# wavelab/libwave

Measured on AMD Instinct MI355X. Metric: point-cloud registrations/sec (1M<->1M pts, ICP), higher is better.
Workload: dtype f32

## Files before the change

### libwave_amd/csrc/wm_bins.hpp

```cpp
#ifndef WM_BINS_HPP
#define WM_BINS_HPP

#include "wm_internal.hpp"

namespace wm {

constexpr int kBinCount = 64;
constexpr int kBinLimbs = 3;
constexpr int kBinComps = kAcc + 1;
constexpr int kBinStride = 32;
constexpr size_t kBinWords = (size_t) kBinCount * kBinLimbs * kBinStride;

__device__ __host__ inline long long bins_to_i64(double v) {
    const double d = v + 6755399441055744.0;
    long long bits;
    __builtin_memcpy(&bits, &d, sizeof(bits));
    return (bits & 0x000FFFFFFFFFFFFFll) - 0x0008000000000000ll;
}

__device__ __host__ inline void bins_split(double x, long long (&l)[kBinLimbs]) {
    const double t2 = trunc(x * 5.9604644775390625e-08);
    const double r1 = fma(-t2, 16777216.0, x);
    const double t1 = trunc(r1 * 65536.0);
    const double r0 = fma(-t1, 1.52587890625e-05, r1);
    const double t0 = trunc(r0 * 72057594037927936.0);
    l[2] = bins_to_i64(t2);
    l[1] = bins_to_i64(t1);
    l[0] = bins_to_i64(t0);
}

constexpr unsigned kBinPoison = kBinStride - 1;
__device__ __forceinline__ void bins_add(long long *bins, unsigned bin, unsigned comp, double x) {
    long long l[kBinLimbs];
    long long *p = bins + (size_t) bin * (kBinLimbs * kBinStride) + comp;
    if (!(fabs(x) < 4611686018427387904.0)) {
        (void) __hip_atomic_fetch_add(bins + (size_t) bin * (kBinLimbs * kBinStride) + kBinPoison, 1ll, __ATOMIC_RELAXED,
                                      __HIP_MEMORY_SCOPE_AGENT);
        return;
    }
    bins_split(x, l);
#pragma unroll
    for (int k = 0; k < kBinLimbs; ++k)
        (void) __hip_atomic_fetch_add(p + k * kBinStride, l[k], __ATOMIC_RELAXED, __HIP_MEMORY_SCOPE_AGENT);
}
__device__ __forceinline__ void bins_add_count(long long *bins, unsigned bin, unsigned comp, long long n) {
    (void) __hip_atomic_fetch_add(bins + (size_t) bin * (kBinLimbs * kBinStride) + comp, n, __ATOMIC_RELAXED, __HIP_MEMORY_SCOPE_AGENT);
}

__device__ __host__ inline double bins_value(long long L0, long long L1, long long L2);

template <int COMPS>
struct BinsLdsT {
    long long part[4][kBinLimbs * COMPS];
    double tot[COMPS];
    unsigned poison;
};
using BinsLds = BinsLdsT<kBinComps>;
template <int THREADS, int COMPS = kBinComps, int VALUES = kAcc>
__device__ __forceinline__ void bins_collect(long long *__restrict__ bins, BinsLdsT<COMPS> &B) {
    static_assert(COMPS < (int) kBinPoison && VALUES <= COMPS, "components below the poison word");
    constexpr int kBinComps = COMPS, kAcc = VALUES;
    constexpr int kWordsPerBin = kBinLimbs * kBinComps;
    constexpr int kGroups = THREADS >= 4 * kWordsPerBin ? 4 : 2;
    static_assert(THREADS >= kGroups * kWordsPerBin && kBinCount % kGroups == 0, "bins per thread group");
    constexpr int kPer = kBinCount / kGroups;
    const unsigned g = threadIdx.x / (unsigned) kWordsPerBin, j = threadIdx.x % (unsigned) kWordsPerBin;
    const unsigned limb = j / (unsigned) kBinComps, comp = j % (unsigned) kBinComps;
    if (threadIdx.x == 0) B.poison = 0u;
    if (g < (unsigned) kGroups) {
        long long v[kPer];
#pragma unroll
        for (int b = 0; b < kPer; ++b)
            v[b] = bins[((size_t) (g * kPer + b) * kBinLimbs + limb) * kBinStride + comp];
        long long t = 0;
#pragma unroll
        for (int b = 0; b < kPer; ++b) t += v[b];
        B.part[g][j] = t;
#pragma unroll
        for (int b = 0; b < kPer; ++b)
            bins[((size_t) (g * kPer + b) * kBinLimbs + limb) * kBinStride + comp] = 0ll;
    }
    __syncthreads();
    if (threadIdx.x < (unsigned) kBinCount) {
        long long *pw = bins + (size_t) threadIdx.x * (kBinLimbs * kBinStride) + kBinPoison;
        if (*pw != 0ll) {
            atomicOr(&B.poison, 1u);
            *pw = 0ll;
        }
    }
    if (threadIdx.x < (unsigned) kBinComps) {
        long long L[kBinLimbs];
#pragma unroll
        for (int l = 0; l < kBinLimbs; ++l) {
            long long t = 0;
#pragma unroll
            for (int gg = 0; gg < kGroups; ++gg) t += B.part[gg][l * kBinComps + threadIdx.x];
            L[l] = t;
        }
        B.tot[threadIdx.x] = threadIdx.x < (unsigned) kAcc ? bins_value(L[0], L[1], L[2]) : (double) L[0];
    }
    __syncthreads();
}

__device__ __host__ inline double bins_value(long long L0, long long L1, long long L2) {
    double term[6];
    const long long L[3] = {L2, L1, L0};
    const double scale[3] = {16777216.0, 1.52587890625e-05, 1.3877787807814457e-17};
    for (int k = 0; k < 3; ++k) {
        const long long hi = L[k] >> 32;
        const long long lo = L[k] - hi * 4294967296ll;
        term[2 * k] = (double) hi * 4294967296.0 * scale[k];
        term[2 * k + 1] = (double) lo * scale[k];
    }
    double s = 0.0, c = 0.0;
    for (int k = 0; k < 6; ++k) {
        const double t = s + term[k];
        const double bb = t - s;
        const double err = (s - (t - bb)) + (term[k] - bb);
        s = t;
        c += err;
    }
    return s + c;
}

}

#endif
```

### libwave_amd/csrc/wm_icp.hip

```cpp
#include "wm_internal.hpp"
#include "wm_icp_step.hpp"
#include "wm_pair_terms.hpp"
#include "wm_bins.hpp"
#include "wm_xchg.hpp"

#include <chrono>
#include <utility>
#include <vector>

#include <float.h>
#include <math.h>
#include <string.h>

#include <new>

namespace wm {

constexpr int kMaxStatBlocks = 256;
constexpr int kStatUnroll = 4;

template <int MODE>
__global__ void __launch_bounds__(kBlock)
    k_icp_stats(const float4 *__restrict__ src, unsigned n,
                const unsigned long long *__restrict__ keys, const float4 *__restrict__ tgt,
                const IcpDevState *__restrict__ st, double *__restrict__ partials, const int *__restrict__ rej) {
    if (st->done) return;
    const int rej_thr = rej ? *rej : 0x7FFFFFFF;
    double a[kAcc];
#pragma unroll
    for (int k = 0; k < kAcc; ++k) a[k] = 0.0;
    const bool slab_on = st->slab_on != 0;
    const float slab_lo = st->slab_lo, slab_hi = st->slab_hi;
    const unsigned stride = gridDim.x * kBlock;
    for (unsigned i0 = blockIdx.x * kBlock + threadIdx.x; i0 < n; i0 += kStatUnroll * stride) {
        float4 p4v[kStatUnroll], q4v[kStatUnroll];
        unsigned long long keyv[kStatUnroll];
#pragma unroll
        for (int u = 0; u < kStatUnroll; ++u) {
            const unsigned i = i0 + u * stride;
            const unsigned ic = i < n ? i : i0;
            p4v[u] = src[ic];
            keyv[u] = keys[ic];
            q4v[u] = tgt[ic];
        }
#pragma unroll
        for (int u = 0; u < kStatUnroll; ++u) {
            if (i0 + u * stride >= n) break;
            float fx, fy, fz;
            xform_pcl(st->Tf, p4v[u].x, p4v[u].y, p4v[u].z, fx, fy, fz);
            if (slab_on && !(fx >= slab_lo && fx < slab_hi)) continue;
            a[17] += 1.0;
            const unsigned long long key = keyv[u];
            if ((unsigned) key == kNoIdx) continue;
            if ((int) (unsigned) (key >> 32) > rej_thr) continue;
            icp_pair_terms<MODE>(fx, fy, fz, q4v[u].x, q4v[u].y, q4v[u].z, __uint_as_float((unsigned) (key >> 32)),
                                 [&](int k, double term) { a[k] += term; });
        }
    }
#pragma unroll
    for (int k = 0; k < kAcc; ++k)
#pragma unroll
        for (int off = 32; off > 0; off >>= 1) a[k] += __shfl_down(a[k], off);
    __shared__ double lds[kBlock / 64][kAcc];
    const int lane = threadIdx.x & 63, wave = threadIdx.x >> 6;
    if (lane == 0)
#pragma unroll
        for (int k = 0; k < kAcc; ++k) lds[wave][k] = a[k];
    __syncthreads();
    if (threadIdx.x < kAcc) {
        double s = 0;
        for (int w = 0; w < kBlock / 64; ++w) s += lds[w][threadIdx.x];
        partials[(size_t) blockIdx.x * kAcc + threadIdx.x] = s;
    }
}

constexpr int kPreRows = 128;
__global__ void __launch_bounds__(kBlock)
    k_reduce_rows(const double *__restrict__ partials, int rows, const IcpDevState *__restrict__ st,
                  double *__restrict__ out) {
    if (st->done) return;
    constexpr int kLanes = kBlock / kAcc;
    __shared__ double lds[kLanes][kAcc];
    const int c = threadIdx.x % kAcc, r = threadIdx.x / kAcc;
    const int r0 = blockIdx.x * kPreRows, r1 = min(r0 + kPreRows, rows);
    if (r < kLanes) {
        double v[(kPreRows + kLanes - 1) / kLanes];
        int k = 0;
#pragma unroll
        for (int b = r0 + r, u = 0; u < (kPreRows + kLanes - 1) / kLanes; b += kLanes, ++u, ++k)
            v[u] = b < r1 ? partials[(size_t) b * kAcc + c] : 0.0;
        double s = 0.0;
#pragma unroll
        for (int u = 0; u < (kPreRows + kLanes - 1) / kLanes; ++u) s += v[u];
        lds[r][c] = s;
    }
    __syncthreads();
    if (threadIdx.x < kAcc) {
        double t = 0.0;
#pragma unroll
        for (int l = 0; l < kLanes; ++l) t += lds[l][threadIdx.x];
        out[(size_t) blockIdx.x * kAcc + threadIdx.x] = t;
    }
}

__global__ void __launch_bounds__(kBlock)
    k_bins_solve(long long *__restrict__ bins, IcpDevState *st, unsigned long long *pub, int pub_slots) {
    __shared__ IcpDevState s_st;
    __shared__ BinsLds s_b;
    const unsigned long long t_start = clock64();
    static_assert(sizeof(IcpDevState) % 4 == 0, "word-wise staging");
    constexpr unsigned kWords = sizeof(IcpDevState) / 4;
    constexpr unsigned kStage = (kWords + kBlock - 1) / kBlock;
    unsigned stage[kStage];
#pragma unroll
    for (unsigned k = 0; k < kStage; ++k) {
        const unsigned w = threadIdx.x + k * kBlock;
        stage[k] = w < kWords ? reinterpret_cast<const unsigned *>(st)[w] : 0u;
    }
    bins_collect<kBlock>(bins, s_b);
#pragma unroll
    for (unsigned k = 0; k < kStage; ++k) {
        const unsigned w = threadIdx.x + k * kBlock;
        if (w < kWords) reinterpret_cast<unsigned *>(&s_st)[w] = stage[k];
    }
    __syncthreads();
    if (s_st.done) return;
    if (threadIdx.x == 0) {
        s_st.dbg[0] = t_start;
        s_st.dbg[1] = clock64();
        double a[kAcc], ex[kStatsLen];
#pragma unroll
        for (int k = 0; k < kAcc; ++k) a[k] = s_b.poison ? 0.0 : s_b.tot[k];
        expand_stats(s_st.mode, a, ex, s_st.changed_mask);
        s_st.local_handled = ex[kStatsLen - 1];
#pragma unroll
        for (int k = 0; k < kStatsLen; ++k) s_st.stats[k] = ex[k];
        s_st.dbg[2] = clock64();
        icp_apply_stats(&s_st, ex, (long long) s_b.tot[kAcc]);
        publish_step(&s_st, pub, pub_slots);
        s_st.dbg[3] = clock64();
    }
    __syncthreads();
    for (unsigned w = threadIdx.x; w < kWords; w += kBlock)
        reinterpret_cast<unsigned *>(st)[w] = reinterpret_cast<const unsigned *>(&s_st)[w];
}

template <int PHASES, int THREADS>
__global__ void __launch_bounds__(THREADS)
    k_reduce_solve(const double *__restrict__ partials, int nblocks, IcpDevState *st,
                   double *stats_io, unsigned long long *pub, int pub_slots, int blk_ext, XchgDev xd, long long *bins) {
    __shared__ IcpDevState s_st;
    const unsigned long long t_start = clock64();
    static_assert(sizeof(IcpDevState) % 4 == 0, "word-wise staging");
    constexpr unsigned kWords = sizeof(IcpDevState) / 4;
    constexpr unsigned kStage = (kWords + THREADS - 1) / THREADS;
    unsigned stage[kStage];
#pragma unroll
    for (unsigned k = 0; k < kStage; ++k) {
        const unsigned w = threadIdx.x + k * THREADS;
        stage[k] = w < kWords ? reinterpret_cast<const unsigned *>(st)[w] : 0u;
    }
    constexpr int kRows = THREADS / kAcc;
    constexpr int kGroups = 8;
    __shared__ double lds[kRows][kAcc];
    __shared__ double lds2[kGroups][kAcc];
    __shared__ double tot[kAcc];
    __shared__ BinsLds s_b;
    const bool from_bins = (PHASES & 1) && bins != nullptr;
    if (from_bins) {
        bins_collect<THREADS>(bins, s_b);
    } else if (PHASES & 1) {
        const int c = threadIdx.x % kAcc, r = threadIdx.x / kAcc;
        if (r < kRows) {
            constexpr int U = 16;
            double s[U];
#pragma unroll
            for (int u = 0; u < U; ++u) s[u] = 0.0;
            for (int b = r; b < nblocks; b += U * kRows) {
                double v[U];
#pragma unroll
                for (int u = 0; u < U; ++u) {
                    const int bb = b + u * kRows;
                    v[u] = bb < nblocks ? partials[(size_t) bb * kAcc + c] : 0.0;
                }
#pragma unroll
                for (int u = 0; u < U; ++u) s[u] += v[u];
            }
#pragma unroll
            for (int w = U / 2; w > 0; w >>= 1)
#pragma unroll
                for (int u = 0; u < w; ++u) s[u] += s[u + w];
            lds[r][c] = s[0];
        }
    }
#pragma unroll
    for (unsigned k = 0; k < kStage; ++k) {
        const unsigned w = threadIdx.x + k * THREADS;
        if (w < kWords) reinterpret_cast<unsigned *>(&s_st)[w] = stage[k];
    }
    if (from_bins) {
        if (threadIdx.x < (unsigned) kAcc) tot[threadIdx.x] = s_b.poison ? 0.0 : s_b.tot[threadIdx.x];
    } else if (PHASES & 1) {
        const int c = threadIdx.x % kAcc;
        __syncthreads();
        if (threadIdx.x < kGroups * kAcc) {
            const int g = threadIdx.x / kAcc;
            double t = 0.0;
            for (int sl = g; sl < kRows; sl += kGroups) t += lds[sl][c];
            lds2[g][c] = t;
        }
        __syncthreads();
        if (threadIdx.x < kAcc) {
            double t = 0.0;
#pragma unroll
            for (int g = 0; g < kGroups; ++g) t += lds2[g][threadIdx.x];
            tot[threadIdx.x] = t;
        }
    }
    __syncthreads();
    if (s_st.done) return;
    __shared__ unsigned s_uns;
    if (threadIdx.x < 64) {
        unsigned v = s_st.cert_unsettled[threadIdx.x];
        s_st.cert_unsettled[threadIdx.x] = 0u;
#pragma unroll
        for (int off = 32; off > 0; off >>= 1) v += (unsigned) __shfl_xor((int) v, off);
        if (threadIdx.x == 0) s_uns = from_bins ? (unsigned) s_b.tot[kAcc] : v;
    }
    if constexpr (PHASES == 7) {
        __shared__ double s_blk[kBlkLen], s_sum[kBlkLen];
        __shared__ unsigned s_half[kXMaxWorld * kXWords], s_ctl[2];
        if (threadIdx.x == 0) {
            double a[kAcc];
#pragma unroll
            for (int k = 0; k < kAcc; ++k) a[k] = tot[k];
            double ex[kStatsLen];
            expand_stats(s_st.mode, a, ex, s_st.changed_mask);
            s_st.local_handled = ex[kStatsLen - 1];
            ex[kStatsLen - 2] = s_st.stripe_finite;
#pragma unroll
            for (int k = 0; k < kStatsLen; ++k) s_blk[k] = ex[k];
            s_blk[kStatsLen] = (double) s_uns;
            s_blk[kStatsLen + 1] = 0.0;
        }
        __syncthreads();
        const bool arrived = xchg_allreduce<THREADS>(xd, s_blk, s_sum, s_half, s_ctl) && s_sum[kStatsLen + 1] == 0.0;
        if (threadIdx.x == 0) {
            s_st.dbg[0] = t_start;
            s_st.dbg[1] = clock64();
            if (!arrived) {
                s_st.xchg_failed = 1;
                s_st.done = 1;
                s_st.converged = 0;
                if (pub) __hip_atomic_store(pub, pack_done_word(1, s_st.iter), __ATOMIC_RELAXED, __HIP_MEMORY_SCOPE_SYSTEM);
            } else {
                double stats[kStatsLen];
#pragma unroll
                for (int k = 0; k < kStatsLen; ++k) stats[k] = s_st.stats[k] = s_sum[k];
                s_st.uns_global = 1;
                s_st.dbg[2] = clock64();
                icp_apply_stats(&s_st, stats, (long long) s_sum[kStatsLen]);
                if (stats_io)
                    for (int k = 0; k < kBlkLen; ++k) stats_io[k] = s_sum[k];
                publish_step(&s_st, pub, pub_slots);
            }
            s_st.dbg[3] = clock64();
        }
    } else if (threadIdx.x == 0) {
        s_st.dbg[0] = t_start;
        s_st.dbg[1] = clock64();
        if (PHASES & 1) {
            double a[kAcc];
#pragma unroll
            for (int k = 0; k < kAcc; ++k) a[k] = tot[k];
            double ex[kStatsLen];
            expand_stats(s_st.mode, a, ex, s_st.changed_mask);
            s_st.local_handled = ex[kStatsLen - 1];
#pragma unroll
            for (int k = 0; k < kStatsLen; ++k) s_st.stats[k] = ex[k];
            if (PHASES == 1 && stats_io) {
                ex[kStatsLen - 2] = s_st.stripe_finite;
#pragma unroll
                for (int k = 0; k < kStatsLen; ++k) stats_io[k] = ex[k];
                if (blk_ext) {
                    stats_io[kStatsLen] = (double) s_uns;
                    stats_io[kStatsLen + 1] = 0.0;
                }
            }
        } else if (stats_io) {
#pragma unroll
            for (int k = 0; k < kStatsLen; ++k) s_st.stats[k] = stats_io[k];
            s_st.uns_global = blk_ext ? 1 : 0;
        }
        if (PHASES & 2) {
            double stats[kStatsLen];
#pragma unroll
            for (int k = 0; k < kStatsLen; ++k) stats[k] = s_st.stats[k];
            s_st.dbg[2] = clock64();
            const long long uns_total = (PHASES == 2 && stats_io && blk_ext) ? (long long) stats_io[kStatsLen] : (long long) s_uns;
            icp_apply_stats(&s_st, stats, uns_total);
            publish_step(&s_st, pub, pub_slots);
        }
        s_st.dbg[3] = clock64();
    }
    __syncthreads();
    for (unsigned w = threadIdx.x; w < kWords; w += THREADS)
        reinterpret_cast<unsigned *>(st)[w] = reinterpret_cast<const unsigned *>(&s_st)[w];
}

__global__ void __launch_bounds__(kBlock) k_xchg_commit(IcpDevState *st, XchgDev xd) {
    __shared__ double s_blk[kBlkLen], s_sum[kBlkLen];
    __shared__ unsigned s_half[kXMaxWorld * kXWords], s_ctl[2];
    if (threadIdx.x < (unsigned) kBlkLen) s_blk[threadIdx.x] = 0.0;
    __syncthreads();
    if (threadIdx.x == 0) {
        s_blk[0] = st->xchg_failed ? 0.0 : 1.0;
        s_blk[kStatsLen + 1] = 1.0;
    }
    __syncthreads();
    const bool arrived = xchg_allreduce<kBlock>(xd, s_blk, s_sum, s_half, s_ctl);
    if (threadIdx.x == 0 && (!arrived || s_sum[0] != (double) xd.world || s_sum[kStatsLen + 1] != (double) xd.world)) {
        st->xchg_failed = 1;
        st->converged = 0;
    }
}

__global__ void __launch_bounds__(kBlock)
    k_unpack_corr(const float4 *__restrict__ src, unsigned n,
                  const unsigned long long *__restrict__ keys, int *__restrict__ match,
                  float *__restrict__ d2) {
    const unsigned i = blockIdx.x * kBlock + threadIdx.x;
    if (i >= n) return;
    const unsigned orig = __float_as_uint(src[i].w);
    const unsigned long long key = keys[i];
    const unsigned idx = (unsigned) key;
    match[orig] = idx == kNoIdx ? -1 : (int) idx;
    d2[orig] = __uint_as_float((unsigned) (key >> 32));
}

static int stat_blocks(size_t n) {
    size_t b = (n + kBlock - 1) / kBlock;
    if (b > kMaxStatBlocks) b = kMaxStatBlocks;
    if (b < 1) b = 1;
    return (int) b;
}

unsigned stat_rows(const wm_ctx *ctx) { return (unsigned) stat_blocks(ctx->n_src); }

int launch_stats(wm_ctx *ctx, int mode, const int *rej) {
    const unsigned n = (unsigned) ctx->n_src;
    const int nb = stat_blocks(n);
    const IcpDevState *st = ctx->d_state.as<IcpDevState>();
    if (mode == WM_ICP_SVD)
        hipLaunchKernelGGL(HIP_KERNEL_NAME(k_icp_stats<WM_ICP_SVD>), dim3(nb), dim3(kBlock), 0,
                           ctx->stream, ctx->src_sorted.as<float4>(), n,
                           ctx->keys.as<unsigned long long>(), ctx->match_pt.as<float4>(), st,
                           ctx->partials.as<double>(), rej);
    else
        hipLaunchKernelGGL(HIP_KERNEL_NAME(k_icp_stats<WM_ICP_GN6>), dim3(nb), dim3(kBlock), 0,
                           ctx->stream, ctx->src_sorted.as<float4>(), n,
                           ctx->keys.as<unsigned long long>(), ctx->match_pt.as<float4>(), st,
                           ctx->partials.as<double>(), rej);
    WM_HIP(ctx, hipGetLastError());
    return WM_OK;
}

int bins_ready(wm_ctx *ctx) {
    if (!ctx->bins.p || ctx->bins_dirty) {
        WM_HIP(ctx, ctx->bins.reserve(kBinWords * sizeof(long long)));
        WM_HIP(ctx, hipMemsetAsync(ctx->bins.p, 0, kBinWords * sizeof(long long), ctx->stream));
        ctx->bins_dirty = false;
    }
    return WM_OK;
// ... 816 lines not shown
```

### libwave_amd/csrc/wm_nn.hip

```cpp
#include "wm_nn_scan.hpp"

namespace wm {

template <int STATS, bool BAL, bool COST = false>
__global__ void __launch_bounds__(64) __attribute__((amdgpu_waves_per_eu(5, 5)))
    k_nn_grid(const LevelsDev lv, const float4 *__restrict__ src, unsigned n,
              IcpDevState *__restrict__ st, float thr_d2, unsigned long long *__restrict__ keys,
              float4 *__restrict__ match_pt, const float4 *__restrict__ tgt_orig,
              float r_light_cells, float lane_lf, float coop_lf, float r0_cells, unsigned chunk_sz,
              double *__restrict__ partials, unsigned *__restrict__ cost_out,
              unsigned long long *__restrict__ phase_out, long long *__restrict__ bins, float rmax) {
    const unsigned lane = threadIdx.x & 63u;
    const unsigned row_c = xcd_remap_chunked(blockIdx.x, max(chunk_sz, 1u)), row_e = xcd_remap(blockIdx.x, gridDim.x);
    const unsigned row = chunk_sz ? row_c : row_e;
    const unsigned i = row * 64u + lane;
    const bool active = i < n;
    const unsigned ic = min(i, n - 1u);
    const float4 p_e = src[ic];
    const unsigned long long prev_e = keys[ic];
    const float4 tp_e = match_pt[ic];
    const NnState S = nn_state(st);
    const int L = lv.n;
    float hl[kMaxLevels];
#pragma unroll
// ... 37 lines not shown
        if (prev != ~0ull) {
            const unsigned pidx = (unsigned) prev;
            r = rmax;
            if (pidx != kNoIdx) {
                const float d2b = canon_d2(qx, qy, qz, tp);
                if (d2b <= thr_d2) {
                    best = seeded = make_key(d2b, pidx);
                    bqx = tp.x;
                    bqy = tp.y;
                    bqz = tp.z;
                    r = fmaxf(__builtin_amdgcn_sqrtf(d2b) * 1.0001f + 1e-6f, 0.05f * h0);
                }
            }
        }
        r = fminf(r, rmax);
        heavy = r > r_light();
    }
    const unsigned long long prof_pro = COST ? clock64() : 0ull;
    if constexpr (BAL) {
        BalLds &L = s_hold.v;
        L.q[lane] = make_float4(qx, qy, qz, 0.f);
        L.seeded[lane] = seeded;
        L.bq[0][lane] = bqx;
        L.bq[1][lane] = bqy;
        L.bq[2][lane] = bqz;
        asm volatile("" ::: "memory");
        bool live = mine && !heavy;
        const bool allow_layered = true;
        bool probing = live && (unsigned) best == kNoIdx && r < rmax;
        if (__ballot(probing) != 0ull) {
            float rp = r0_cells * h0;
            for (int rung = 0; rung < 16 && __ballot(probing) != 0ull; ++rung) {
                int lp = 0;
#pragma unroll
                for (int k = 1; k < kMaxLevels; ++k) lp += (k < L_levels && hl[k] <= rp) ? 1 : 0;
                const GridDev g = lv.g[lp];
                unsigned cand;
                const bool empty = probe_box_empty(g, probing, qx, qy, qz, rp, cand);
                const bool hit = probing && !empty;
                const f4v ct = ((gp_f4) g.pts)[hit ? cand : 0u];
                if (hit) {
                    const float d2c = canon_d2v(qx, qy, qz, ct);
                    const float rc = fmaxf(__builtin_amdgcn_sqrtf(d2c) * 1.0001f + 1e-6f, 0.05f * h0);
                    if (d2c <= thr_d2 && rc <= r_light()) {
                        best = make_key(d2c, __float_as_uint(ct.w));
                        r = fminf(rc, rmax);
                    }
                }
                if (probing) {
                    if constexpr (COST) cost += ((cost >> 28) & 7u) < 7u ? 1u << 28 : 0u;
                    if (empty) {
                        r = nn_grow_radius(best, 0.f, r, rmax);
                        heavy = r > r_light();
                        live = !heavy;
                    }
                    probing = empty && live && r < rmax;
                }
                rp = fminf(2.0f * rp, rmax);
            }
        }
        for (int pass = 0; pass < 32 && __ballot(live) != 0ull; ++pass) {
            const int l = nn_level_for(hl, L_levels, lane_lf, r);
            const unsigned long long lv_mask = __ballot(live);
            const int l0 = __builtin_amdgcn_readlane(l, __ffsll((long long) lv_mask) - 1);
            float margin;
            if (__ballot(live && l != l0) == 0ull) {
                const GridDev g = lv.g[l0];
                best = scan_box_bal<COST, kBalRowChunk>(g, live, qx, qy, qz, r, best, &margin, L, lane, allow_layered, g.pts, cost, prof);
            } else {
                const GridDev g = lv.g[l];
                L.base[lane] = (unsigned long long) g.pts;
                best = scan_box_bal<COST, kBalRowChunk>(g, live, qx, qy, qz, r, best, &margin, L, lane, allow_layered, nullptr, cost, prof);
            }
            if (live) {
                if constexpr (COST) cost += ((cost >> 24) & 15u) < 15u ? 1u << 24 : 0u;
                const float bd2 = __uint_as_float((unsigned) (best >> 32));
                if (nn_certified(margin, bd2, thr_d2)) {
                    live = false;
                } else {
                    r = nn_grow_radius(best, bd2, r, rmax);
                    heavy = r > r_light();
                    live = !heavy;
                }
            }
        }
    } else if (mine) {
        for (int pass = 0; !heavy && pass < 32; ++pass) {
            const int l = nn_level_for(hl, L_levels, lane_lf, r);
            const GridDev g = lv.g[l];
            float margin;
            best = scan_box<COST>(g, qx, qy, qz, r, best, &margin, s_runs, lane, have_prev, cost);
            if constexpr (COST) cost += ((cost >> 24) & 15u) < 15u ? 1u << 24 : 0u;
            const float bd2 = __uint_as_float((unsigned) (best >> 32));
            if (nn_certified(margin, bd2, thr_d2)) break;
            r = nn_grow_radius(best, bd2, r, rmax);
            heavy = r > r_light();
        }
    }
    const unsigned long long prof_pass = COST ? clock64() : 0ull;
    unsigned long long todo = __ballot(heavy);
    const unsigned n_heavy = __popcll(todo);
    float seed = 0.f;
    while (todo) {
        const int sl = __ffsll((long long) todo) - 1;
        todo &= todo - 1;
        const float ux = rl_f(qx, sl), uy = rl_f(qy, sl), uz = rl_f(qz, sl);
        float ur = rl_f(r, sl);
        unsigned long long ub = ((unsigned long long) rl_u((unsigned) (best >> 32), sl) << 32) |
                                rl_u((unsigned) best, sl);
        if ((unsigned) ub == kNoIdx && seed > ur) ur = fminf(seed, rmax);
        for (int pass = 0; pass < 64; ++pass) {
            const int l = nn_level_for(hl, L_levels, coop_lf, ur);
            const GridDev g = lv.g[l];
            float margin;
            ub = coop_scan_box(g, ux, uy, uz, ur, ub, lane, &margin);
            const float bd2 = __uint_as_float((unsigned) (ub >> 32));
            if (nn_certified(margin, bd2, thr_d2)) break;
            if (ur >= rmax) break;
            ur = nn_grow_radius(ub, bd2, ur, rmax);
        }
        seed = ((unsigned) ub != kNoIdx) ? 1.25f * sqrtf(__uint_as_float((unsigned) (ub >> 32))) : ur;
        if ((int) lane == sl) best = ub;
    }
    const unsigned lane_e = __builtin_amdgcn_mbcnt_hi(~0u, __builtin_amdgcn_mbcnt_lo(~0u, 0u));
    const unsigned i_e = BAL ? row * 64u + lane_e : i;
    if constexpr (BAL) {
        asm volatile("" ::: "memory");
        BalLds &L = s_hold.v;
        seeded = L.seeded[lane_e];
        bqx = L.bq[0][lane_e];
        bqy = L.bq[1][lane_e];
        bqz = L.bq[2][lane_e];
    }
    if (mine) {
        st_u64(&keys[i_e], best);
        if (best != seeded && (unsigned) best != kNoIdx) {
            const f4v c = ((gp_f4) tgt_orig)[(unsigned) best];
            bqx = c.x;
            bqy = c.y;
            bqz = c.z;
        }
        if (!(best == seeded && (unsigned) best != kNoIdx))
            st_f4(&match_pt[i_e], bqx, bqy, bqz, __uint_as_float((unsigned) best));
    }
    if (lane == 0 && n_heavy) atomicAdd(&st->queue_count[1], n_heavy);
    const unsigned long long prof_store = COST ? clock64() : 0ull;
    if constexpr (COST) {
        if (active) cost_out[i_e] = mine ? (cost | (heavy ? 0x80000000u : 0u)) : 0u;
    }
    if constexpr (STATS >= 0) {
        double a[kAcc];
        icp_terms<STATS>(a, mine, (unsigned) best != kNoIdx, qx, qy, qz, bqx, bqy, bqz,
                         __uint_as_float((unsigned) (best >> 32)),
                         (unsigned) best != (unsigned) seeded && (i_e & st->changed_mask) == 0u);
        acc_halve<kAcc, 32>(a, lane);
        const int comp = acc_comp_of_lane(lane);
        if (comp >= 0) {
            if (bins) bins_add(bins, row % (unsigned) kBinCount, (unsigned) comp, a[0]);
            else st_f64(&partials[(size_t) row * kAcc + comp], a[0]);
        }
    }
    if constexpr (COST) {
        if (lane_e == 0 && phase_out) {
            const unsigned long long t_end = clock64();
            atomicAdd(&phase_out[0], prof[0]);
            atomicAdd(&phase_out[1], prof[1]);
            atomicAdd(&phase_out[2], prof[2]);
            atomicAdd(&phase_out[3], prof_pro - prof_start);
            atomicAdd(&phase_out[4], prof_pass - prof_pro);
            atomicAdd(&phase_out[5], prof_store - prof_pass);
            atomicAdd(&phase_out[6], t_end - prof_store);
            atomicAdd(&phase_out[7], 1ull);
        }
    }
}

constexpr int kBruteTile = 1024;

__global__ void __launch_bounds__(kBlock) k_init_keys(unsigned long long *keys, unsigned n,
                                                       const IcpDevState *st, float thr_d2) {
    if (st->done) return;
    const unsigned i = blockIdx.x * kBlock + threadIdx.x;
    if (i < n) keys[i] = make_key(thr_d2, kNoIdx);
}

__global__ void __launch_bounds__(kBlock)
    k_nn_brute(const float4 *__restrict__ tgt, unsigned m, const float4 *__restrict__ src,
               unsigned n, const IcpDevState *__restrict__ st, float thr_d2,
               unsigned long long *__restrict__ keys) {
    if (st->done) return;
    __shared__ float4 tile[kBruteTile];
    const unsigned i = blockIdx.x * kBlock + threadIdx.x;
    const unsigned per = (m + gridDim.y - 1) / gridDim.y;
    const unsigned m0 = blockIdx.y * per, m1 = min(m0 + per, m);
    float qx = 0, qy = 0, qz = 0;
    if (i < n) xform_pcl(st->Tf, src[i].x, src[i].y, src[i].z, qx, qy, qz);
    const bool mine = !(st->slab_on && !(qx >= st->slab_lo && qx < st->slab_hi));
    unsigned long long best = make_key(thr_d2, kNoIdx);
    for (unsigned t0 = m0; t0 < m1; t0 += kBruteTile) {
        const unsigned cnt = min((unsigned) kBruteTile, m1 - t0);
        __syncthreads();
        for (unsigned k = threadIdx.x; k < cnt; k += kBlock) tile[k] = tgt[t0 + k];
        __syncthreads();
        for (unsigned k = 0; k < cnt; ++k) {
            const float4 t = tile[k];
            const unsigned long long key = make_key(canon_d2(qx, qy, qz, t), __float_as_uint(t.w));
            best = key < best ? key : best;
        }
    }
    if (i < n && mine && best < make_key(thr_d2, kNoIdx)) atomicMin(&keys[i], best);
}

__global__ void __launch_bounds__(kBlock)
    k_fill_match(const unsigned long long *__restrict__ keys, unsigned n,
                 const float4 *__restrict__ tgt, const IcpDevState *__restrict__ st,
                 float4 *__restrict__ match_pt) {
    if (st->done) return;
    const unsigned i = blockIdx.x * kBlock + threadIdx.x;
    if (i >= n) return;
    const unsigned idx = (unsigned) keys[i];
    match_pt[i] = idx == kNoIdx ? make_float4(0.f, 0.f, 0.f, __uint_as_float(kNoIdx)) : tgt[idx];
}

static float threshold_below(double max_corr, bool strict) {
    const double m2 = max_corr * max_corr;
    if (!(m2 < 3.0e38)) return 3.0e38f;
    float f = (float) m2;
    if (strict ? (double) f >= m2 : (double) f > m2) f = nextafterf(f, 0.0f);
    return f;
}
float threshold_d2(double max_corr) { return threshold_below(max_corr, false); }
float threshold_d2_strict(double max_corr) { return threshold_below(max_corr, true); }

int nn_sums_target(wm_ctx *ctx, int stats_mode, bool use_bins, unsigned blocks, long long **bins, unsigned *rows_out) {
    *bins = nullptr;
    if (stats_mode >= 0 && use_bins) {
        if (!ctx->bins.p) return WM_ERR_STATE;
        *bins = ctx->bins.as<long long>();
    } else if (stats_mode >= 0) {
        WM_HIP(ctx, ctx->partials.reserve((size_t) blocks * kAcc * sizeof(double)));
        if (rows_out) *rows_out = blocks;
    }
    return WM_OK;
}

template <int STATS, bool BAL, bool COST = false>
static void launch_nn_grid_t(wm_ctx *ctx, unsigned blocks, float thr_d2, unsigned xcd_chunk, long long *bins = nullptr) {
    hipLaunchKernelGGL(HIP_KERNEL_NAME(k_nn_grid<STATS, BAL, COST>), dim3(blocks), dim3(64), 0, ctx->stream,
                       ctx->levels_dev, ctx->src_sorted.as<float4>(), (unsigned) ctx->n_src,
                       ctx->d_state.as<IcpDevState>(), thr_d2, ctx->keys.as<unsigned long long>(),
                       ctx->match_pt.as<float4>(), ctx->tgt_orig.as<float4>(), ctx->tune_r_light,
                       ctx->tune_lane_lf, ctx->tune_coop_lf, ctx->tune_r0, xcd_chunk, ctx->partials.as<double>(),
                       ctx->cost_log.p ? ctx->cost_log.as<unsigned>() + (size_t) ctx->cost_log_iter * ctx->n_src : nullptr,
                       ctx->phase_log.p ? ctx->phase_log.as<unsigned long long>() + 8 * (size_t) ctx->cost_log_iter : nullptr, bins,
                       sqrtf(thr_d2) * 1.0001f + 1e-6f);
}

int launch_nn_grid(wm_ctx *ctx, float thr_d2, hipEvent_t ev0, hipEvent_t ev1, hipEvent_t ev2,
                   int stats_mode, unsigned *rows_out, bool use_bins) {
    const unsigned n = (unsigned) ctx->n_src;
    if (rows_out) *rows_out = 0;
    if (n == 0) return WM_OK;
    unsigned blocks = (n + 63u) / 64u;
    blocks = (blocks + 7u) & ~7u;
    unsigned xcd_chunk = 0;
    if (ctx->tune_xcd_chunk > 0 && blocks >= 32u * (unsigned) ctx->tune_xcd_chunk) {
        xcd_chunk = (unsigned) ctx->tune_xcd_chunk;
        const unsigned m = 8u * xcd_chunk;
        blocks = (blocks + m - 1u) / m * m;
    }
    long long *bins = nullptr;
    const int rc = nn_sums_target(ctx, stats_mode, use_bins, blocks, &bins, rows_out);
    if (rc != WM_OK) return rc;
    const bool bal = ctx->tune_nn_balanced && ctx->n_tgt_input < (1u << 26) - 8u;
    if (ev0) WM_HIP(ctx, hipEventRecord(ev0, ctx->stream));
    if (stats_mode == WM_ICP_SVD && ctx->cost_log.p && ctx->cost_log_iter < ctx->cost_log_cap) {
        if (bal) launch_nn_grid_t<WM_ICP_SVD, true, true>(ctx, blocks, thr_d2, xcd_chunk, bins);
        else launch_nn_grid_t<WM_ICP_SVD, false, true>(ctx, blocks, thr_d2, xcd_chunk, bins);
        ctx->cost_log_iter++;
    } else if (stats_mode < 0) {
        if (bal) launch_nn_grid_t<-1, true>(ctx, blocks, thr_d2, xcd_chunk);
        else launch_nn_grid_t<-1, false>(ctx, blocks, thr_d2, xcd_chunk);
    } else if (stats_mode == WM_ICP_SVD) {
        if (bal) launch_nn_grid_t<WM_ICP_SVD, true>(ctx, blocks, thr_d2, xcd_chunk, bins);
        else launch_nn_grid_t<WM_ICP_SVD, false>(ctx, blocks, thr_d2, xcd_chunk, bins);
    } else {
        if (bal) launch_nn_grid_t<WM_ICP_GN6, true>(ctx, blocks, thr_d2, xcd_chunk, bins);
        else launch_nn_grid_t<WM_ICP_GN6, false>(ctx, blocks, thr_d2, xcd_chunk, bins);
    }
    if (ev1) WM_HIP(ctx, hipEventRecord(ev1, ctx->stream));
    if (ev2) WM_HIP(ctx, hipEventRecord(ev2, ctx->stream));
    WM_HIP(ctx, hipGetLastError());
    return WM_OK;
}

int launch_nn_brute(wm_ctx *ctx, float thr_d2, hipEvent_t ev0, hipEvent_t ev1) {
    const unsigned n = (unsigned) ctx->n_src, m = (unsigned) ctx->n_tgt_input;
    if (n == 0) return WM_OK;
    const IcpDevState *st = ctx->d_state.as<IcpDevState>();
    unsigned long long *keys = ctx->keys.as<unsigned long long>();
    const unsigned bx = (n + kBlock - 1) / kBlock;
    unsigned splits = 1;
    if (m > 0) {
        splits = (2048 + bx - 1) / bx;
        const unsigned max_splits = (m + kBruteTile - 1) / kBruteTile;
        if (splits > max_splits) splits = max_splits;
        if (splits < 1) splits = 1;
// ... 16 lines not shown
```

### libwave_amd/csrc/wm_plane.hip

```cpp
#include "wm_internal.hpp"
#include "wm_icp_step.hpp"
#include "wm_bins.hpp"
#include "wm_gicp_dev.hpp"
#include "wm_pair_terms.hpp"

#include <string.h>

namespace wm {

constexpr int kNrmBlock = 64;
template <int K>
__global__ void __launch_bounds__(kNrmBlock) __attribute__((amdgpu_waves_per_eu(K <= 10 ? 6 : (K <= 12 ? 5 : 1))))
    k_normals(GridDev g, const float4 *__restrict__ qpts, unsigned n, const float4 *__restrict__ orig, unsigned n_orig, int k,
              float4 *__restrict__ out, float r0_cells) {
    __shared__ uint2 s_runs[kKnnRows * kNrmBlock];
    const unsigned i = blockIdx.x * kNrmBlock + threadIdx.x;
    if (i >= n) return;
    const float4 q = qpts[i];
    const unsigned slot = __float_as_uint(q.w);
    if (slot >= n_orig) return;
    if (!(q.x == q.x)) {
        out[slot] = make_float4(0.f, 0.f, 0.f, 0.f);
        return;
    }
// ... 60 lines not shown
                            float4 *out) {
    return knn_ladder(k, [&](auto K) { return launch_normals<decltype(K)::value>(ctx, g, q, n, orig, n_orig, k, out); });
}

int plane_normal_k(int k) { return k == 0 ? kPlaneDefaultK : k; }

int plane_target_normals(wm_ctx *ctx, int k) {
    k = plane_normal_k(k);
    if (k < 3 || k > 32) return WM_ERR_ARG;
    if (ctx->plane_nrm_valid && ctx->plane_nrm_k == k) return WM_OK;
    if ((size_t) k > ctx->n_tgt) return WM_NOT_CONVERGED;
    if (!ctx->levels[0].built) WM_TRY(ensure_levels(ctx, -1.0));
    const size_t n_in = ctx->n_tgt_input;
    WM_HIP(ctx, ctx->plane_nrm.reserve((n_in + 1) * sizeof(float4)));
    if (ctx->n_tgt != n_in) WM_HIP(ctx, hipMemsetAsync(ctx->plane_nrm.p, 0, n_in * sizeof(float4), ctx->stream));
    const GridDev &g = ctx->levels[0].d;
    WM_TRY(launch_normals_k(ctx, g, g.pts, ctx->n_tgt, ctx->tgt_orig.as<float4>(), n_in, k, ctx->plane_nrm.as<float4>()));
    ctx->plane_nrm_valid = true;
    ctx->plane_nrm_k = k;
    return WM_OK;
}

constexpr int kPlaneComps = 29;
constexpr int kPlaneUnroll = 4;
constexpr int kPlaneMaxBlocks = 1024;
static_assert(kGnG + 6 == kPlaneComps && kPlaneComps < (int) kBinPoison, "the GN layout inside a bin's limb row");

__global__ void __launch_bounds__(kBlock)
    k_plane_stats(const float4 *__restrict__ src, unsigned n, const unsigned long long *__restrict__ keys,
                  const float4 *__restrict__ match_pt, const float4 *__restrict__ normals, unsigned n_normals,
                  const IcpDevState *__restrict__ st, long long *__restrict__ bins, const int *__restrict__ rej) {
    if (st->done) return;
    const int rej_thr = rej ? *rej : 0x7FFFFFFF;
    double a[kPlaneComps];
#pragma unroll
    for (int k = 0; k < kPlaneComps; ++k) a[k] = 0.0;
    float T[12];
#pragma unroll
    for (int k = 0; k < 12; ++k) T[k] = st->Tf[k];
    const unsigned stride = gridDim.x * kBlock;
    for (unsigned i0 = blockIdx.x * kBlock + threadIdx.x; i0 < n; i0 += kPlaneUnroll * stride) {
        float4 pv[kPlaneUnroll], qv[kPlaneUnroll], nv[kPlaneUnroll];
        unsigned long long keyv[kPlaneUnroll];
#pragma unroll
        for (int u = 0; u < kPlaneUnroll; ++u) {
            const unsigned i = i0 + u * stride;
            const unsigned ic = i < n ? i : i0;
            pv[u] = src[ic];
            keyv[u] = keys[ic];
            qv[u] = match_pt[ic];
        }
#pragma unroll
        for (int u = 0; u < kPlaneUnroll; ++u) {
            const unsigned idx = (unsigned) keyv[u];
            nv[u] = normals[idx < n_normals ? idx : 0u];
        }
#pragma unroll
        for (int u = 0; u < kPlaneUnroll; ++u) {
            if (i0 + u * stride >= n) break;
            const unsigned long long key = keyv[u];
            const unsigned idx = (unsigned) key;
            if (idx >= n_normals) continue;
            if ((int) (unsigned) (key >> 32) > rej_thr) continue;
            const float4 p4 = pv[u];
            float fx, fy, fz;
            xform_pcl(T, p4.x, p4.y, p4.z, fx, fy, fz);
            a[kGnN] += 1.0;
            a[kGnSd2] += (double) __uint_as_float((unsigned) (key >> 32));
            const float4 n4 = nv[u];
            if (n4.x == 0.f && n4.y == 0.f && n4.z == 0.f) continue;
            const double px = fx, py = fy, pz = fz;
            const double J[6] = {(double) n4.x, (double) n4.y, (double) n4.z,
                                 py * (double) n4.z - pz * (double) n4.y,
                                 pz * (double) n4.x - px * (double) n4.z,
                                 px * (double) n4.y - py * (double) n4.x};
            const double r = J[0] * (px - (double) qv[u].x) + J[1] * (py - (double) qv[u].y) + J[2] * (pz - (double) qv[u].z);
            int k = kGnH;
#pragma unroll
            for (int i = 0; i < 6; ++i)
#pragma unroll
                for (int j = i; j < 6; ++j) a[k++] += J[i] * J[j];
#pragma unroll
            for (int i = 0; i < 6; ++i) a[kGnG + i] += J[i] * r;
        }
    }
#pragma unroll
    for (int k = 0; k < kPlaneComps; ++k)
#pragma unroll
        for (int off = 32; off > 0; off >>= 1) a[k] += __shfl_down(a[k], off);
    __shared__ double lds[kBlock / 64][kPlaneComps];
    const int lane = threadIdx.x & 63, wave = threadIdx.x >> 6;
    if (lane == 0)
#pragma unroll
        for (int k = 0; k < kPlaneComps; ++k) lds[wave][k] = a[k];
    __syncthreads();
    if (threadIdx.x < kPlaneComps) {
        double s = 0;
#pragma unroll
        for (int w = 0; w < kBlock / 64; ++w) s += lds[w][threadIdx.x];
        bins_add(bins, blockIdx.x % (unsigned) kBinCount, threadIdx.x, s);
    }
}

int plane_bins_ready(wm_ctx *ctx) {
    WM_HIP(ctx, ctx->plane_bins.reserve(kBinWords * sizeof(long long)));
    WM_HIP(ctx, hipMemsetAsync(ctx->plane_bins.p, 0, kBinWords * sizeof(long long), ctx->stream));
    return WM_OK;
}

int launch_plane_stats(wm_ctx *ctx, const int *rej) {
    const unsigned n = (unsigned) ctx->n_src;
    if (n == 0) return WM_OK;
    if (!ctx->plane_bins.p || !ctx->plane_nrm_valid) return WM_ERR_STATE;
    unsigned blocks = (n + kBlock * kPlaneUnroll - 1) / (kBlock * kPlaneUnroll);
    if (blocks > (unsigned) kPlaneMaxBlocks) blocks = kPlaneMaxBlocks;
    hipLaunchKernelGGL(k_plane_stats, dim3(blocks), dim3(kBlock), 0, ctx->stream, ctx->src_sorted.as<float4>(), n,
                       ctx->keys.as<unsigned long long>(), ctx->match_pt.as<float4>(), ctx->plane_nrm.as<float4>(),
                       (unsigned) ctx->n_tgt_input, ctx->d_state.as<IcpDevState>(), ctx->plane_bins.as<long long>(), rej);
    WM_HIP(ctx, hipGetLastError());
    return WM_OK;
}

constexpr double kPlanePivotTol = 1e-12;
__host__ __device__ inline bool plane_degenerate(const double *st) {
    double A[36], L[36], dmax = 0.0;
    int k = 0;
    for (int i = 0; i < 6; ++i)
        for (int j = i; j < 6; ++j) {
            A[i * 6 + j] = A[j * 6 + i] = st[kGnH + k];
            ++k;
        }
    for (int i = 0; i < 6; ++i) dmax = fmax(dmax, A[i * 7]);
    if (!(dmax > 0.0)) return true;
    for (int i = 0; i < 6; ++i)
        for (int j = 0; j <= i; ++j) {
            double s = A[i * 6 + j];
            for (int m = 0; m < j; ++m) s -= L[i * 6 + m] * L[j * 6 + m];
            if (i == j) {
                if (!(s > kPlanePivotTol * dmax)) return true;
                L[i * 6 + i] = sqrt(s);
            } else {
                L[i * 6 + j] = s / L[j * 6 + j];
            }
        }
    return false;
}

__global__ void __launch_bounds__(kBlock)
    k_plane_solve(long long *__restrict__ bins, IcpDevState *st, unsigned long long *pub, int pub_slots, unsigned n_src, int solve) {
    __shared__ IcpDevState s_st;
    __shared__ BinsLdsT<kPlaneComps> s_b;
    static_assert(sizeof(IcpDevState) % 4 == 0, "word-wise staging");
    constexpr unsigned kWords = sizeof(IcpDevState) / 4;
    for (unsigned w = threadIdx.x; w < kWords; w += kBlock) reinterpret_cast<unsigned *>(&s_st)[w] = reinterpret_cast<const unsigned *>(st)[w];
    bins_collect<kBlock, kPlaneComps, kPlaneComps>(bins, s_b);
    if (s_st.done) return;
    if (threadIdx.x == 0) {
        double ex[kStatsLen];
#pragma unroll
        for (int k = 0; k < kStatsLen; ++k) ex[k] = 0.0;
        if (!s_b.poison)
            for (int k = 0; k < kPlaneComps; ++k) ex[k] = s_b.tot[k];
        ex[kStatsLen - 1] = (double) n_src;
        s_st.local_handled = ex[kStatsLen - 1];
        for (int k = 0; k < kStatsLen; ++k) s_st.stats[k] = ex[k];
        if (solve) {
            if (ex[kGnN] >= 3.0 && plane_degenerate(ex)) {
                for (int k = 0; k < 12; ++k) s_st.Tf_search[k] = s_st.Tf[k];
                s_st.n_corr = (int) ex[kGnN];
                s_st.mse = ex[kGnSd2] / ex[kGnN];
                s_st.deferred_total += s_st.queue_count[1];
                for (int l = 0; l <= kMaxLevels; ++l) s_st.queue_count[l] = 0;
                for (int k = 0; k < 64; ++k) s_st.cert_unsettled[k] = 0u;
                s_st.state = WM_CONV_DEGENERATE;
                s_st.converged = 0;
                s_st.done = 1;
            } else {
                icp_apply_stats(&s_st, ex);
            }
            publish_step(&s_st, pub, pub_slots);
        }
    }
    __syncthreads();
    for (unsigned w = threadIdx.x; w < kWords; w += kBlock) reinterpret_cast<unsigned *>(st)[w] = reinterpret_cast<const unsigned *>(&s_st)[w];
}

int launch_plane_solve(wm_ctx *ctx, unsigned long long *pub, int pub_slots, int solve) {
    hipLaunchKernelGGL(k_plane_solve, dim3(1), dim3(kBlock), 0, ctx->stream, ctx->plane_bins.as<long long>(),
                       ctx->d_state.as<IcpDevState>(), pub, pub_slots, (unsigned) ctx->n_src, solve);
    WM_HIP(ctx, hipGetLastError());
    return WM_OK;
}

}

using namespace wm;

extern "C" int wm_estimate_normals(wm_ctx *ctx, int which, int k, void *normals_out, int out_mem) {
    if (!ctx || (which != 0 && which != 1) || !normals_out || (out_mem != WM_MEM_HOST && out_mem != WM_MEM_DEVICE)) return WM_ERR_ARG;
    k = plane_normal_k(k);
    if (k < 3 || k > 32) return WM_ERR_ARG;
    if (ctx->n_src_input == 0 || ctx->n_tgt_input == 0) return WM_ERR_STATE;
    WM_HIP(ctx, hipSetDevice(ctx->device));
    WM_TRY(finalize_clouds(ctx));
    const float4 *res = nullptr;
    size_t n_out = 0;
    if (which == 1) {
        WM_TRY(plane_target_normals(ctx, k));
        res = ctx->plane_nrm.as<float4>();
        n_out = ctx->n_tgt_input;
    } else {
        if ((size_t) k > ctx->n_src) return WM_NOT_CONVERGED;
        n_out = ctx->n_src_input;
        WM_HIP(ctx, ctx->plane_nrm_src.reserve((n_out + 1) * sizeof(float4)));
        WM_HIP(ctx, hipMemsetAsync(ctx->plane_nrm_src.p, 0, n_out * sizeof(float4), ctx->stream));
        WM_TRY(source_grid(ctx));
        WM_TRY(launch_normals_k(ctx, ctx->src_grid.d, ctx->src_sorted.as<float4>(), ctx->n_src, ctx->src_orig.as<float4>(), n_out, k,
                                ctx->plane_nrm_src.as<float4>()));
        res = ctx->plane_nrm_src.as<float4>();
    }
    if (out_mem == WM_MEM_DEVICE) {
        WM_HIP(ctx, hipMemcpyAsync(normals_out, res, n_out * sizeof(float4), hipMemcpyDeviceToDevice, ctx->stream));
        WM_HIP(ctx, hipStreamSynchronize(ctx->stream));
        return WM_OK;
    }
    return copy_to_caller(ctx, normals_out, res, n_out * sizeof(float4));
}
```

Baseline: 295.5.

## Move bin zeroing off the collect path and ballot the poison check

The bin accumulator is now only read inside bins_collect. The poison words are loaded up front alongside the limb loads and reduced with a wave ballot instead of a second pass with LDS atomics. Zeroing moves to a new bins_reset that uses 16-byte vector stores from the non-solving waves, running after the done check and in parallel with thread 0's solve. The plane solve also stages its state loads in registers so they overlap the bin collection, and asm hints keep kernel arguments in scalar registers. One kernel now reads changed_mask from the shared copy rather than from global state. Risk: bins are not cleared when the state is already done, so a later launch could see stale sums.

New measurement: 295.2. Within noise of the previous version (-0.1%).

```diff
diff --git a/libwave_amd/csrc/wm_bins.hpp b/libwave_amd/csrc/wm_bins.hpp
--- a/libwave_amd/csrc/wm_bins.hpp
+++ b/libwave_amd/csrc/wm_bins.hpp
@@ -57,8 +57,9 @@
 };
 using BinsLds = BinsLdsT<kBinComps>;
 template <int THREADS, int COMPS = kBinComps, int VALUES = kAcc>
-__device__ __forceinline__ void bins_collect(long long *__restrict__ bins, BinsLdsT<COMPS> &B) {
+__device__ __forceinline__ void bins_collect(const long long *__restrict__ bins, BinsLdsT<COMPS> &B) {
     static_assert(COMPS < (int) kBinPoison && VALUES <= COMPS, "components below the poison word");
+    static_assert(THREADS >= kBinCount && kBinCount == 64, "the poison words' readers are the lanes of wave 0");
     constexpr int kBinComps = COMPS, kAcc = VALUES;
     constexpr int kWordsPerBin = kBinLimbs * kBinComps;
     constexpr int kGroups = THREADS >= 4 * kWordsPerBin ? 4 : 2;
@@ -66,7 +67,7 @@
     constexpr int kPer = kBinCount / kGroups;
     const unsigned g = threadIdx.x / (unsigned) kWordsPerBin, j = threadIdx.x % (unsigned) kWordsPerBin;
     const unsigned limb = j / (unsigned) kBinComps, comp = j % (unsigned) kBinComps;
-    if (threadIdx.x == 0) B.poison = 0u;
+    const long long pw = bins[(size_t) (threadIdx.x % (unsigned) kBinCount) * (kBinLimbs * kBinStride) + kBinPoison];
     if (g < (unsigned) kGroups) {
         long long v[kPer];
 #pragma unroll
@@ -76,18 +77,11 @@
 #pragma unroll
         for (int b = 0; b < kPer; ++b) t += v[b];
         B.part[g][j] = t;
-#pragma unroll
-        for (int b = 0; b < kPer; ++b)
-            bins[((size_t) (g * kPer + b) * kBinLimbs + limb) * kBinStride + comp] = 0ll;
     }
+    const bool raised = threadIdx.x < (unsigned) kBinCount && pw != 0ll;
+    const unsigned long long any_raised = __ballot(raised);
+    if (threadIdx.x == 0) B.poison = any_raised != 0ull ? 1u : 0u;
     __syncthreads();
-    if (threadIdx.x < (unsigned) kBinCount) {
-        long long *pw = bins + (size_t) threadIdx.x * (kBinLimbs * kBinStride) + kBinPoison;
-        if (*pw != 0ll) {
-            atomicOr(&B.poison, 1u);
-            *pw = 0ll;
-        }
-    }
     if (threadIdx.x < (unsigned) kBinComps) {
         long long L[kBinLimbs];
 #pragma unroll
@@ -100,6 +94,15 @@
         B.tot[threadIdx.x] = threadIdx.x < (unsigned) kAcc ? bins_value(L[0], L[1], L[2]) : (double) L[0];
     }
     __syncthreads();
+}
+
+template <int THREADS>
+__device__ __forceinline__ void bins_reset(long long *__restrict__ bins) {
+    typedef long long ll2v __attribute__((ext_vector_type(2)));
+    static_assert(THREADS > 64 && kBinWords % 2 == 0, "waves beside the one that solves; whole 16-byte stores");
+    if (threadIdx.x >= 64u)
+        for (unsigned w = threadIdx.x - 64u; w < (unsigned) (kBinWords / 2); w += (unsigned) THREADS - 64u)
+            reinterpret_cast<ll2v *>(bins)[w] = ll2v{0ll, 0ll};
 }
 
 __device__ __host__ inline double bins_value(long long L0, long long L1, long long L2) {
diff --git a/libwave_amd/csrc/wm_icp.hip b/libwave_amd/csrc/wm_icp.hip
--- a/libwave_amd/csrc/wm_icp.hip
+++ b/libwave_amd/csrc/wm_icp.hip
@@ -107,6 +107,7 @@
     k_bins_solve(long long *__restrict__ bins, IcpDevState *st, unsigned long long *pub, int pub_slots) {
     __shared__ IcpDevState s_st;
     __shared__ BinsLds s_b;
+    asm volatile("" ::"s"(bins), "s"(st), "s"(pub), "s"(pub_slots));
     const unsigned long long t_start = clock64();
     static_assert(sizeof(IcpDevState) % 4 == 0, "word-wise staging");
     constexpr unsigned kWords = sizeof(IcpDevState) / 4;
@@ -125,6 +126,7 @@
     }
     __syncthreads();
     if (s_st.done) return;
+    bins_reset<kBlock>(bins);
     if (threadIdx.x == 0) {
         s_st.dbg[0] = t_start;
         s_st.dbg[1] = clock64();
@@ -150,6 +152,8 @@
     k_reduce_solve(const double *__restrict__ partials, int nblocks, IcpDevState *st,
                    double *stats_io, unsigned long long *pub, int pub_slots, int blk_ext, XchgDev xd, long long *bins) {
     __shared__ IcpDevState s_st;
+    asm volatile("" ::"s"(partials), "s"(nblocks), "s"(st), "s"(stats_io), "s"(pub), "s"(pub_slots), "s"(blk_ext), "s"(bins),
+                 "s"(xd.peer), "s"(xd.mine), "s"(xd.world), "s"(xd.rank), "s"(xd.timeout_ms));
     const unsigned long long t_start = clock64();
     static_assert(sizeof(IcpDevState) % 4 == 0, "word-wise staging");
     constexpr unsigned kWords = sizeof(IcpDevState) / 4;
@@ -219,6 +223,7 @@
     }
     __syncthreads();
     if (s_st.done) return;
+    if (from_bins) bins_reset<THREADS>(bins);
     __shared__ unsigned s_uns;
     if (threadIdx.x < 64) {
         unsigned v = s_st.cert_unsettled[threadIdx.x];
diff --git a/libwave_amd/csrc/wm_nn.hip b/libwave_amd/csrc/wm_nn.hip
--- a/libwave_amd/csrc/wm_nn.hip
+++ b/libwave_amd/csrc/wm_nn.hip
@@ -213,7 +213,7 @@
         double a[kAcc];
         icp_terms<STATS>(a, mine, (unsigned) best != kNoIdx, qx, qy, qz, bqx, bqy, bqz,
                          __uint_as_float((unsigned) (best >> 32)),
-                         (unsigned) best != (unsigned) seeded && (i_e & st->changed_mask) == 0u);
+                         (unsigned) best != (unsigned) seeded && (i_e & S.changed_mask) == 0u);
         acc_halve<kAcc, 32>(a, lane);
         const int comp = acc_comp_of_lane(lane);
         if (comp >= 0) {
diff --git a/libwave_amd/csrc/wm_plane.hip b/libwave_amd/csrc/wm_plane.hip
--- a/libwave_amd/csrc/wm_plane.hip
+++ b/libwave_amd/csrc/wm_plane.hip
@@ -236,9 +236,23 @@
     __shared__ BinsLdsT<kPlaneComps> s_b;
     static_assert(sizeof(IcpDevState) % 4 == 0, "word-wise staging");
     constexpr unsigned kWords = sizeof(IcpDevState) / 4;
-    for (unsigned w = threadIdx.x; w < kWords; w += kBlock) reinterpret_cast<unsigned *>(&s_st)[w] = reinterpret_cast<const unsigned *>(st)[w];
+    asm volatile("" ::"s"(bins), "s"(st), "s"(pub), "s"(pub_slots), "s"(n_src), "s"(solve));
+    constexpr unsigned kStage = (kWords + kBlock - 1) / kBlock;
+    unsigned stage[kStage];
+#pragma unroll
+    for (unsigned k = 0; k < kStage; ++k) {
+        const unsigned w = threadIdx.x + k * kBlock;
+        stage[k] = w < kWords ? reinterpret_cast<const unsigned *>(st)[w] : 0u;
+    }
     bins_collect<kBlock, kPlaneComps, kPlaneComps>(bins, s_b);
+#pragma unroll
+    for (unsigned k = 0; k < kStage; ++k) {
+        const unsigned w = threadIdx.x + k * kBlock;
+        if (w < kWords) reinterpret_cast<unsigned *>(&s_st)[w] = stage[k];
+    }
+    __syncthreads();
     if (s_st.done) return;
+    bins_reset<kBlock>(bins);
     if (threadIdx.x == 0) {
         double ex[kStatsLen];
 #pragma unroll
```
